# sdiehl/sonic

Hardware: AMD Instinct MI355X
Metric: prove() proofs/sec (higher is better)
Workload: dtype u32 limbs (Fq 12x32, Fr 8x32 Montgomery); 1 GPU; prove(): rndCircuit n=2^18, Q=2, SRS d=2^21 (d=8n >= 7n, Protocol.hs:54); n=262144, Q=2, d=2097152, process_group=none (plain single-process run), legs=headline only (the other legs: --full)

## Files before the change

sonic_amd/csrc/msm.hip:

```cpp
#include <string.h>
#include <stdexcept>
#include "internal.hpp"
#include "g1_quad.hpp"
#include "endo.hpp"

namespace sonic {

#ifndef SONIC_PART_LOW_BITS
#define SONIC_PART_LOW_BITS 8
#endif
constexpr int PART_LOW_BITS = SONIC_PART_LOW_BITS;
#ifndef SONIC_PART_TILE
#define SONIC_PART_TILE 1024
#endif
constexpr int PART_TILE = SONIC_PART_TILE;
constexpr uint32_t PASS1_GRID = 1024;
constexpr uint32_t PART_SORT_GRID = 2048;
#ifndef SONIC_PART_SORT_THREADS
#define SONIC_PART_SORT_THREADS 1024
#endif
constexpr int PART_SORT_THREADS = SONIC_PART_SORT_THREADS;
#ifndef SONIC_PART_SCATTER_THREADS
#define SONIC_PART_SCATTER_THREADS 512
#endif
// ... 36 lines not shown
  p.nseg = p.NB / K;
}

MsmPlan msm_plan(long n, bool fold) {
  MsmPlan p;
  p.fold = fold;
  int lg = 0;
  while ((1L << (lg + 1)) <= n) lg++;
  int c = lg - 4;
  if (c < 4) c = 4;
  if (c > 16) c = 16;
  if (g_window_override >= 4 && g_window_override <= 16) c = g_window_override;
  p.c = c;
  p.W = ((fold ? 255 : 256) + c - 1) / c;
  p.Wb = p.W;
  p.table_stride = 0;
  plan_finish(p, n);
  return p;
}

MsmPlan msm_plan_tables(long n, int c, int W, long table_stride, bool endo) {
  MsmPlan p;
  p.fold = true;
  p.endo = endo;
  p.bits = endo ? ENDO_BITS : 255;
  p.c = c;
  p.W = W;
  p.Wb = 1;
  p.table_stride = table_stride;
  plan_finish(p, n);
  return p;
}

void MsmWorkspace::reserve(long n, const MsmPlan& pl, int k) {
  const size_t sets = (size_t)k * pl.Wb;
  size_t M = sets * pl.NB;
  size_t NW = (size_t)n * pl.W;
  const size_t part_hn = (size_t)ceil_div((long)pl.Wb * pl.NB, 1L << PART_LOW_BITS) * (size_t)(ceil_div(n, PART_TILE) + k);
  count.ensure((2 * part_hn + 4) * 4);
  off.ensure((M + 1) * 4);
  digits.ensure(NW * 8);
  entries.ensure(NW * 4);
  buckets.ensure(M * sizeof(G1XYZZ));
  segres.ensure((sets * pl.nseg + sets * (pl.nseg / 256 + 1) + 2) * sizeof(G1XYZZ));
  scan_tmp.ensure((part_hn / 2048 + 4) * 4);
  order.ensure((M + 1) * 4);
  size_t max_heavy = NW / pl.heavy_threshold + 1;
  heavy_meta.ensure(sizeof(HeavyMeta) + max_heavy * sizeof(HeavyRec));
  heavy_partial.ensure((max_heavy + HEAVY_GRID + 1) * sizeof(G1XYZZ));
}

__device__ __forceinline__ bool fr_gt_half(const Fr& s) {
  constexpr uint32_t half[8] = FR_HALF;
#pragma unroll
  for (int i = 7; i >= 0; i--) {
    if (s.l[i] > half[i]) return true;
    if (s.l[i] < half[i]) return false;
  }
  return false;
}

__device__ __forceinline__ uint32_t block_exclusive_scan_256(uint32_t v, uint32_t* sh, uint32_t* total);
__device__ __forceinline__ uint32_t size_class(uint32_t sz) { return 255u - (sz < 255u ? sz : 255u); }


struct MsmBatchDev {
  int k;
  int bits;
  int slot_off[MSM_MAX_JOBS];
  int slot_form;
  uint32_t tile0[MSM_MAX_JOBS + 1];
  const char* points[MSM_MAX_JOBS];
  uint32_t pt_stride;
  long tstride[MSM_MAX_JOBS];
  const Fr* scalars[MSM_MAX_JOBS];
  long n[MSM_MAX_JOBS];
  MsmSlot* slot[MSM_MAX_JOBS];
// ... 523 lines not shown
      acc = k == (uint32_t)q ? c : g1q_add(acc, c, cr);
    }
    reinterpret_cast<Fq*>(&sh[q])[cr] = acc;
    __syncthreads();
    for (int sp = 8; sp >= 1; sp >>= 1) {
      if (q < sp && (uint32_t)(q + sp) < r.npart) {
        Fq* pa = reinterpret_cast<Fq*>(&sh[q]) + cr;
        *pa = g1q_add(*pa, reinterpret_cast<const Fq*>(&sh[q + sp])[cr], cr);
      }
      __syncthreads();
    }
    if (threadIdx.x < 4) reinterpret_cast<Fq*>(&buckets[r.bucket])[threadIdx.x] = reinterpret_cast<const Fq*>(&sh[0])[threadIdx.x];
    __syncthreads();
  }
}

#ifndef SONIC_SEGMENTS_LDS_TOT
#define SONIC_SEGMENTS_LDS_TOT 1
#endif
struct LdsPoint {
  uint32_t* base;
  __device__ __forceinline__ void store(const G1XYZZ& p) const {
    const uint32_t* w = reinterpret_cast<const uint32_t*>(&p);
#pragma unroll
    for (int k = 0; k < 48; k++) base[k * 256] = w[k];
  }
  __device__ __forceinline__ G1XYZZ load() const {
    G1XYZZ p;
    uint32_t* w = reinterpret_cast<uint32_t*>(&p);
#pragma unroll
    for (int k = 0; k < 48; k++) w[k] = base[k * 256];
    return p;
  }
};
__global__ __launch_bounds__(256, SONIC_SEGMENTS_LDS_TOT ? 2 : 1) void k_bucket_segments(const G1XYZZ* __restrict__ buckets, int W, int NB, int K, int nseg, int sg_base,
                                                        G1XYZZ* __restrict__ segres) {
#if SONIC_SEGMENTS_LDS_TOT
  __shared__ uint32_t tot_sh[48 * 256];
  const LdsPoint tl{tot_sh + threadIdx.x};
#endif
  int t = blockIdx.x * blockDim.x + threadIdx.x;
  if (t >= W * nseg) return;
  const int w = t / nseg, sl = t % nseg;
  const G1XYZZ* B = buckets + (size_t)w * NB + (size_t)sl * K;
  const int sg = sg_base + sl;
  const int k0 = sg * K;
  G1XYZZ run = G1XYZZ::inf();
#if SONIC_SEGMENTS_LDS_TOT
  tl.store(G1XYZZ::inf());
  for (int j = K - 1; j >= 0; j--) {
    run = g1_add(run, B[j]);
    tl.store(g1_add(tl.load(), run));
  }
#else
  G1XYZZ tot = G1XYZZ::inf();
  for (int j = K - 1; j >= 0; j--) {
    run = g1_add(run, B[j]);
    tot = g1_add(tot, run);
  }
#endif
  G1XYZZ acc = G1XYZZ::inf();
  bool have_multiple = false;
  if (nseg % 64 == 0 && sg_base % 64 == 0) {
    const uint32_t hi = __builtin_amdgcn_readfirstlane((uint32_t)sg >> 6), lo = (uint32_t)sg & 63u;
    for (int i = 31 - __clz((int)(hi | 1u)); i >= 0; i--) {
      acc = g1_dbl(acc);
      if ((hi >> i) & 1u) acc = g1_add(acc, run);
    }
    for (int i = 5; i >= 0; i--) {
      acc = g1_dbl(acc);
      if ((lo >> i) & 1u) acc = g1_add(acc, run);
    }
    for (int s = K; s > 1; s >>= 1) acc = g1_dbl(acc);
    have_multiple = true;
  } else if (k0) {
    acc = g1_mul_small(run, (uint32_t)k0);
    have_multiple = true;
  }
#if SONIC_SEGMENTS_LDS_TOT
  G1XYZZ tot = tl.load();
#endif
  if (have_multiple) tot = g1_add(tot, acc);
  segres[t] = tot;
}

__global__ __launch_bounds__(256, 2) void k_window_sum(const G1XYZZ* __restrict__ segres, int W, int c, int nseg, const MsmBatchDev batch) {
  __shared__ G1XYZZ sh[256];
  const int w = blockIdx.x % W;
  MsmSlot* slot = batch.slot[blockIdx.x / W];
  segres += (size_t)(blockIdx.x - w) * nseg;
  G1XYZZ acc = G1XYZZ::inf();
  for (int s = threadIdx.x; s < nseg; s += 256) acc = g1_add(acc, segres[(size_t)w * nseg + s]);
  sh[threadIdx.x] = acc;
  __syncthreads();
  for (int s = 128; s >= 1; s >>= 1) {
    if ((int)threadIdx.x < s) sh[threadIdx.x] = g1_add(sh[threadIdx.x], sh[threadIdx.x + s]);
    __syncthreads();
  }
  if (threadIdx.x == 0) {
    G1XYZZ r = sh[0];
    r.x = fp_canonical(r.x); r.y = fp_canonical(r.y); r.zz = fp_canonical(r.zz); r.zzz = fp_canonical(r.zzz);
    slot->win[w] = r;
    if (w == 0) { slot->W = W; slot->c = c; slot->pad0 = 0; slot->pad1 = 0; }
  }
}

__global__ __launch_bounds__(256, 2) void k_group_sum(const G1XYZZ* __restrict__ in, long n_in, int group, G1XYZZ* __restrict__ out) {
  __shared__ G1XYZZ sh[256];
  const long base = (long)blockIdx.x * group;
  G1XYZZ acc = G1XYZZ::inf();
  for (long s = threadIdx.x; s < group && base + s < n_in; s += 256) acc = g1_add(acc, in[base + s]);
  sh[threadIdx.x] = acc;
  __syncthreads();
  for (int s = 128; s >= 1; s >>= 1) {
    if ((int)threadIdx.x < s) sh[threadIdx.x] = g1_add(sh[threadIdx.x], sh[threadIdx.x + s]);
    __syncthreads();
  }
  if (threadIdx.x == 0) out[blockIdx.x] = sh[0];
}

constexpr int TREE_BLOCK_LOG = 10;
constexpr int TREE_MID_LOG = 14;
#ifndef SONIC_TREE_LATENCY_MAX
#define SONIC_TREE_LATENCY_MAX (1L << 17)
#endif
constexpr long TREE_LATENCY_MAX_BUCKETS = SONIC_TREE_LATENCY_MAX;
constexpr int TREE_LATENCY_BLOCK_LOG = 7, TREE_LATENCY_MID_LOG = 12;

__device__ __forceinline__ void tree_item(G1XYZZ* __restrict__ Z, size_t s0, int m, uint32_t it) {
  const uint32_t pair = it / (uint32_t)m, comp = it % (uint32_t)m;
  const size_t s = s0 + ((size_t)pair << m);
  const size_t pos = comp == 0 ? 0 : (size_t)1 << (comp - 1);
  const size_t h = (size_t)1 << (m - 1);
  Z[s + pos] = g1_add(Z[s + pos], Z[s + h + pos]);
// ... 23 lines not shown
  const bool leaf_in_registers = quads < 32;
  if (!leaf_in_registers) {
    tree_level(Z, s0, 1, 1u << (LB - 1), quads);
    __syncthreads();
    tree_level(Z, s0, 2, 2u << (LB - 2), quads);
  } else if (threadIdx.x < nthreads) {
    G1XYZZ* b = Z + s0 + 4 * (size_t)threadIdx.x;
    const G1XYZZ odd = g1_add(b[1], b[3]);
    const G1XYZZ p23 = g1_add(b[2], b[3]);
    b[3] = odd;
    const G1XYZZ tot = g1_add(g1_add(b[0], b[1]), p23);
    b[2] = p23;
    b[0] = tot;
    b[1] = b[3];
  }
  for (int m = 3; m <= LB; m++) {
    __syncthreads();
    tree_level(Z, s0, m, (uint32_t)m << (LB - m), quads);
  }
}

template <int THREADS>
__global__ __launch_bounds__(THREADS, THREADS == 256 ? 2 : 1) void k_bucket_tree_levels(G1XYZZ* __restrict__ Z, int span_log, int m_lo, int m_hi, int final_L,
                                                               uint32_t tot_mul, int quads, const MsmBatchDev batch) {
  const size_t s0 = (size_t)blockIdx.x << span_log;
  for (int m = m_lo; m <= m_hi; m++) {
    if (m > m_lo) __syncthreads();
    tree_level(Z, s0, m, (uint32_t)m << (span_log - m), quads);
  }
  if (final_L > 0) {
    __syncthreads();
    MsmSlot* slot = batch.slot[blockIdx.x];
    const int off = batch.slot_off[blockIdx.x];
    if ((int)threadIdx.x <= final_L) {
      G1XYZZ r = Z[s0 + ((int)threadIdx.x == final_L ? 0 : (size_t)1 << threadIdx.x)];
      r.x = fp_canonical(r.x); r.y = fp_canonical(r.y); r.zz = fp_canonical(r.zz); r.zzz = fp_canonical(r.zzz);
      slot->win[off + threadIdx.x] = r;
    }
    if (threadIdx.x == 0 && off == 0) { slot->W = final_L; slot->c = 1; slot->pad0 = (int)tot_mul; slot->pad1 = batch.slot_form; }
  }
}


static void bucket_tree_enqueue(hipStream_t st, G1XYZZ* Z, int sets, int L, uint32_t tot_mul, const MsmBatchDev& batch) {
  if (((long)sets << L) <= TREE_LATENCY_MAX_BUCKETS) {
    constexpr int all_quads = 1 << 20;
    const int LB = L < TREE_LATENCY_BLOCK_LOG ? L : TREE_LATENCY_BLOCK_LOG;
    LAUNCH(k_bucket_tree_block, (uint32_t)sets << (L - LB), 256, 0, st, Z, LB, all_quads);
    int done = LB;
    if (L > TREE_LATENCY_MID_LOG) {
      LAUNCH(k_bucket_tree_levels<512>, (uint32_t)sets << (L - TREE_LATENCY_MID_LOG), 512, 0, st, Z, TREE_LATENCY_MID_LOG, done + 1, TREE_LATENCY_MID_LOG, 0, 0u, all_quads, batch);
      done = TREE_LATENCY_MID_LOG;
    }
    LAUNCH(k_bucket_tree_levels<512>, (uint32_t)sets, 512, 0, st, Z, L, done + 1, L, L, tot_mul, all_quads, batch);
    return;
  }
  const int LB = L < TREE_BLOCK_LOG ? L : TREE_BLOCK_LOG;
  constexpr int quads = 2;
  LAUNCH(k_bucket_tree_block, (uint32_t)sets << (L - LB), 256, 0, st, Z, LB, quads);
  int done = LB;
  if (L > done) {
    const int mid = L < TREE_MID_LOG ? L : TREE_MID_LOG;
    if (mid < L) {
      LAUNCH(k_bucket_tree_levels<256>, (uint32_t)sets << (L - mid), 256, 0, st, Z, mid, done + 1, mid, 0, 0u, quads, batch);
      done = mid;
    }
  }
  LAUNCH(k_bucket_tree_levels<256>, (uint32_t)sets, 256, 0, st, Z, L, done + 1, L, L, tot_mul, quads, batch);
}

G1XYZZ msm_finish_host(const MsmSlot& s) {
  const int W = s.W, c = s.c;
  G1XYZZ acc = G1XYZZ::inf();
  if (s.pad1 == 1 || s.pad1 == 2) {
    auto bitsum = [&](int off) {
      G1XYZZ a = G1XYZZ::inf();
      for (int w = W - 1; w >= 0; w--) {
        G1XYZZ win;
        memcpy(&win, &s.win[off + w], sizeof win);
        a = g1_add(g1_dbl(a), win);
      }
      G1XYZZ tot;
      memcpy(&tot, &s.win[off + W], sizeof tot);
      const uint32_t mul = (uint32_t)s.pad0;
      return g1_add(a, mul == 1 ? tot : g1_mul_small(tot, mul));
    };
    if (s.pad1 == 1) return bitsum(0);
    return g1_add(bitsum(0), g1_endo(bitsum(MSM_ENDO_SLOT_OFFSET)));
  }
  for (int w = W - 1; w >= 0; w--) {
    G1XYZZ win;
    memcpy(&win, &s.win[w], sizeof win);
    if (w == W - 1) { acc = win; continue; }
    for (int j = 0; j < c; j++) acc = g1_dbl(acc);
    acc = g1_add(acc, win);
  }
  return acc;
}
bool msm_can_batch(const MsmPlan& pl) { return pl.Wb == 1 && pl.NB >= (1 << PART_LOW_BITS); }

__global__ __launch_bounds__(256) void k_endo_split(const Fr* __restrict__ sc, long n, int mont, Fr* __restrict__ s1, Fr* __restrict__ s2) {
  const long i = (long)blockIdx.x * blockDim.x + threadIdx.x;
  if (i >= n) return;
  Fr s = sc[i];
  if (mont) s = fp_from_mont(s);
  Fr a, b;
  endo_split(s, a, b);
  s1[i] = a; s2[i] = b;
}

void msm_enqueue_batch(hipStream_t st, MsmWorkspace& ws, const MsmPlan& pl, const MsmJob* jobs, int k, bool scalars_mont, G1XYZZ* ext_buckets) {
  if (k < 1 || k > MSM_MAX_JOBS) throw std::runtime_error("msm_enqueue_batch: 1..MSM_MAX_JOBS jobs");
  if (ext_buckets && (k != 1 || pl.Wb != 1)) throw std::runtime_error("msm_enqueue_batch: bucket hand-off needs one job over a shared bucket set");
  if (k > 1 && !msm_can_batch(pl)) throw std::runtime_error("msm_enqueue_batch: plan cannot be batched");
  MsmJob split_jobs[MSM_MAX_JOBS];
  bool fold = pl.fold;
  if (pl.endo) {
    if (ext_buckets) { set_error("the bucket hand-off of a bucket-sharded MSM needs the full window tables (this SRS holds endomorphism tables)"); throw HipFail{SONIC_ERR_INVALID_ARG}; }
    if (2 * k > MSM_MAX_JOBS) {
      const int h = MSM_MAX_JOBS / 2;
      for (int j0 = 0; j0 < k; j0 += h) msm_enqueue_batch(st, ws, pl, jobs + j0, k - j0 < h ? k - j0 : h, scalars_mont, nullptr);
      return;
    }
    long n_all = 0;
    for (int j = 0; j < k; j++) n_all += jobs[j].n;
    ws.endo_scalars.ensure(sizeof(Fr) * 2 * (size_t)(n_all > 0 ? n_all : 1));
    Fr* halves = ws.endo_scalars.as<Fr>();
    for (int j = 0; j < k; j++) {
      Fr* s1 = halves; Fr* s2 = halves + jobs[j].n;
      halves += 2 * jobs[j].n;
      if (jobs[j].n > 0) LAUNCH(k_endo_split, ceil_div(jobs[j].n, 256), 256, 0, st, jobs[j].scalars, jobs[j].n, (int)scalars_mont, s1, s2);
// ... 76 lines not shown
      const long mean = nmax * pl.W / (P > 0 ? P : 1);
      stage_cap = 2048;
      while (stage_cap < 32768 && (long)stage_cap < mean + mean / 2) stage_cap *= 2;
    }
    LAUNCH(k_part_sort, nparts < PART_SORT_GRID ? nparts : PART_SORT_GRID, PART_SORT_THREADS, (size_t)stage_cap * 4, st, batch, (const uint2*)ws.digits.as<uint2>(),
           (const uint32_t*)hbase, (const uint32_t*)total, hn, P, jobstride, off, ws.entries.as<uint32_t>(), hm->class_hist, stage_cap);
  }
  LAUNCH(k_border_place, ceil_div((long)M, 2048), 256, 0, st, (const uint32_t*)off, (uint32_t)M, (const uint32_t*)hm->class_hist, hm->class_cursor,
         ws.order.as<uint32_t>());
  const int accum_block = (pl.accum_block == 64 || pl.accum_block == 128) ? pl.accum_block : 256;
  static const int split_env = getenv("SONIC_ACCUM_LANES") ? atoi(getenv("SONIC_ACCUM_LANES")) : 0;
  const int lanes_per_bucket = split_env == 1 ? 1 : (M <= 65536 ? 4 : (M <= 131072 ? 2 : 1));
  if (lanes_per_bucket == 4)
    LAUNCH(k_bucket_accum_split<4>, ceil_div(4 * (long)M, 256), 256, 0, st, batch, jobstride, (const uint32_t*)ws.entries.as<uint32_t>(),
           (const uint32_t*)off, (const uint32_t*)ws.order.as<uint32_t>(), (uint32_t)M, pl.heavy_threshold, buckets, hm, hrecs);
  else if (lanes_per_bucket == 2)
    LAUNCH(k_bucket_accum_split<2>, ceil_div(2 * (long)M, 256), 256, 0, st, batch, jobstride, (const uint32_t*)ws.entries.as<uint32_t>(),
           (const uint32_t*)off, (const uint32_t*)ws.order.as<uint32_t>(), (uint32_t)M, pl.heavy_threshold, buckets, hm, hrecs);
  else
  LAUNCH(k_bucket_accum, ceil_div((long)M, accum_block), accum_block, 0, st, batch, jobstride, (const uint32_t*)ws.entries.as<uint32_t>(),
         (const uint32_t*)off, (const uint32_t*)ws.order.as<uint32_t>(), (uint32_t)M, pl.heavy_threshold, buckets, hm, hrecs);
  LAUNCH(k_heavy_accum, HEAVY_GRID, HEAVY_THREADS, 0, st, batch, jobstride, (const uint32_t*)ws.entries.as<uint32_t>(), (const uint32_t*)off,
         (const HeavyMeta*)hm, hrecs, ws.heavy_partial.as<G1XYZZ>());
  LAUNCH(k_heavy_finish, HEAVY_GRID / 2, 64, 0, st, (const HeavyMeta*)hm, (const HeavyRec*)hrecs,
         (const G1XYZZ*)ws.heavy_partial.as<G1XYZZ>(), buckets);
  if (ext_buckets) return;
  const int sets = k * pl.Wb;
  if ((pl.tree && pl.Wb == 1 && pl.NB >= 4) || pl.endo) {
    int L = 0;
    while ((1 << L) < pl.NB) L++;
    bucket_tree_enqueue(st, ws.buckets.as<G1XYZZ>(), sets, L, 1u, batch);
    return;
  }
  LAUNCH(k_bucket_segments, ceil_div((long)sets * pl.nseg, 256), 256, 0, st, (const G1XYZZ*)ws.buckets.as<G1XYZZ>(), sets,
         pl.NB, pl.K, pl.nseg, 0, ws.segres.as<G1XYZZ>());
  if (pl.nseg > 4096) {
    const int group = 256, ngroups = pl.nseg / group;
    G1XYZZ* part = ws.segres.as<G1XYZZ>() + (size_t)sets * pl.nseg;
    LAUNCH(k_group_sum, sets * ngroups, 256, 0, st, (const G1XYZZ*)ws.segres.as<G1XYZZ>(), (long)sets * pl.nseg, group, part);
    LAUNCH(k_window_sum, sets, 256, 0, st, (const G1XYZZ*)part, pl.Wb, pl.c, ngroups, batch);
  } else {
    LAUNCH(k_window_sum, sets, 256, 0, st, (const G1XYZZ*)ws.segres.as<G1XYZZ>(), pl.Wb, pl.c, pl.nseg, batch);
  }
}

__global__ __launch_bounds__(256, 1) void k_sum_slices(const G1XYZZ* __restrict__ slices, int k, long len, G1XYZZ* __restrict__ out) {
  const long i = (long)blockIdx.x * blockDim.x + threadIdx.x;
  if (i >= len) return;
  G1XYZZ acc = slices[i];
  for (int s = 1; s < k; s++) acc = g1_add(acc, slices[(size_t)s * len + i]);
  out[i] = acc;
}

void msm_reduce_slices_enqueue(hipStream_t st, MsmWorkspace& ws, const G1XYZZ* d_slices, int k, long len, long base, int c, MsmSlot* d_slot) {
  (void)c;
  if (k < 1 || len < 4 || len % MSM_SLICE_QUANTUM || base % MSM_SLICE_QUANTUM || base + len >= (1L << 31))
    throw std::runtime_error("msm_reduce_slices_enqueue: slice length and base must be multiples of MSM_SLICE_QUANTUM");
  int L = 2;
  while (((long)1 << L) < len) L++;
  const long P = (long)1 << L;
  ws.buckets.ensure((size_t)P * sizeof(G1XYZZ));
  if (P > len) HIP_OK(hipMemsetAsync(ws.buckets.as<G1XYZZ>() + len, 0, (size_t)(P - len) * sizeof(G1XYZZ), st));
  LAUNCH(k_sum_slices, ceil_div(len, 256), 256, 0, st, d_slices, k, len, ws.buckets.as<G1XYZZ>());
  MsmBatchDev b1;
  memset(&b1, 0, sizeof b1);
  b1.k = 1;
  b1.bits = 255;
  b1.slot_form = 1;
  b1.slot[0] = d_slot;
  bucket_tree_enqueue(st, ws.buckets.as<G1XYZZ>(), 1, L, (uint32_t)(base + 1), b1);
}

void msm_enqueue(hipStream_t st, MsmWorkspace& ws, const MsmPlan& pl, PointArray d_points, const Fr* d_scalars,
                 long n, bool scalars_mont, MsmSlot* d_slot) {
  MsmJob job{d_points, d_scalars, n, d_slot};
// ... 5 lines not shown
```

sonic_amd/csrc/msm.hpp:

```cpp
#pragma once
#include "common.hpp"
#include "g1.hpp"
#include "g1_host.hpp"

namespace sonic {

HD int msm_even_width(int W, int w, int bits = 255) { return bits / W + (w < bits % W ? 1 : 0); }
HD int msm_even_shift(int W, int w, int bits = 255) { const int base = bits / W, extra = bits % W; return w * base + (w < extra ? w : extra); }

struct MsmPlan {
  int c;
  int W;
  int Wb;
  long table_stride;
  int NB;
  int K;
  int nseg;
  uint32_t heavy_threshold;
  int accum_block = 256;
  bool tree = true;
  bool endo = false;
  int bits = 255;
  bool fold;
};
MsmPlan msm_plan(long n, bool fold = true);
MsmPlan msm_plan_tables(long n, int c, int W, long table_stride, bool endo = false);
void msm_plan_set_segment(MsmPlan& p, int K);

constexpr int MSM_MAX_WINDOWS = 64;
constexpr long MSM_TABLE_MAX_TERMS = 1L << 26;
constexpr int MSM_TABLE_MAX_WINDOWS = 32;
constexpr long MSM_MAX_TERMS = 1L << 31;

struct MsmSlot {
  int W, c, pad0, pad1;
  G1XYZZ win[MSM_MAX_WINDOWS];
};

struct MsmWorkspace {
  DevBuf count, off, digits, entries, buckets, segres, scan_tmp, order, heavy_meta, heavy_partial, endo_scalars;
  void reserve(long n, const MsmPlan& pl, int k = 1);
};

void msm_enqueue(hipStream_t st, MsmWorkspace& ws, const MsmPlan& pl, PointArray d_points,
                 const Fr* d_scalars, long n, bool scalars_mont, MsmSlot* d_slot);

constexpr int MSM_MAX_JOBS = 16;
constexpr int MSM_ENDO_SLOT_OFFSET = 32;
struct MsmJob { PointArray points; const Fr* scalars; long n; MsmSlot* slot; long table_stride = 0; };
bool msm_can_batch(const MsmPlan& pl);
void msm_enqueue_batch(hipStream_t st, MsmWorkspace& ws, const MsmPlan& pl, const MsmJob* jobs, int k, bool scalars_mont,
                       G1XYZZ* ext_buckets = nullptr);
constexpr long MSM_SLICE_QUANTUM = 16384;
void msm_reduce_slices_enqueue(hipStream_t st, MsmWorkspace& ws, const G1XYZZ* d_slices, int k, long len, long base, int c, MsmSlot* d_slot);

G1XYZZ msm_finish_host(const MsmSlot& s);
int msm_window_override();
void msm_set_window_override(int c);

}
```

sonic_amd/csrc/msm_api.hip:

```cpp
#include <string.h>
#include <condition_variable>
#include <memory>
#include <string>
#include <vector>
#include "srs_handle.hpp"

using namespace sonic;

extern "C" {

int sonic_msm_set_window(int c) { msm_set_window_override(c); return SONIC_OK; }

int sonic_msm_plan(const sonic_srs_t* srs, int64_t n, int* window_bits, int* windows, int* bucket_sets) {
  if (!srs || n < 0) return SONIC_ERR_INVALID_ARG;
  if (n >= MSM_MAX_TERMS) { set_error("MSM of %ld terms: at most 2^31 - 1 (entry encoding)", (long)n); return SONIC_ERR_INVALID_ARG; }
  MsmPlan pl = srs_msm_plan(srs, n);
  if (window_bits) *window_bits = pl.c;
  if (windows) *windows = pl.W;
  if (bucket_sets) *bucket_sets = pl.Wb;
  return SONIC_OK;
}

int sonic_msm_g1(const uint8_t* points, const uint8_t* scalars, int64_t n, uint8_t out_g1[96]) {
  API_BEGIN
// ... 333 lines not shown
      }
  if (exchange) return sonic_g1_sum_dev_partials(blobs.data(), world, out_g1);
  G1XYZZ acc = G1XYZZ::inf();
  for (int r = 0; r < world; r++) acc = g1_add(acc, partial[(size_t)r]);
  g1_canonical_bytes_host(acc, out_g1);
  return SONIC_OK;
}

int sonic_msm_g1_srs_multi_dev(const sonic_srs_t* const* srs, int world, int basis, const int64_t* e0, const void* const* d_scalars, const int64_t* n, int mode,
                               uint8_t out_g1[96]) {
  if (!e0 || !d_scalars || !n) return SONIC_ERR_INVALID_ARG;
  try { return msm_multi(srs, world, basis, e0, d_scalars, nullptr, n, mode, out_g1); }
  catch (const std::exception& e) { set_error("%s", e.what()); return SONIC_ERR_HIP; }
}
int sonic_msm_g1_srs_multi(const sonic_srs_t* const* srs, int world, int basis, int64_t e0, const uint8_t* scalars, int64_t n, int mode, uint8_t out_g1[96]) {
  if (world < 1 || world > 64 || n < 0 || (n > 0 && !scalars)) return SONIC_ERR_INVALID_ARG;
  std::vector<int64_t> e((size_t)world), cnt((size_t)world);
  std::vector<const uint8_t*> hs((size_t)world);
  for (int r = 0; r < world; r++) {
    const int64_t lo = n * r / world, hi = n * (r + 1) / world;
    e[(size_t)r] = e0 + lo; cnt[(size_t)r] = hi - lo; hs[(size_t)r] = scalars + 32 * (size_t)lo;
  }
  try { return msm_multi(srs, world, basis, e.data(), nullptr, hs.data(), cnt.data(), mode, out_g1); }
  catch (const std::exception& e2) { set_error("%s", e2.what()); return SONIC_ERR_HIP; }
}

static_assert(sizeof(MsmSlot) == SONIC_G1_DEV_PARTIAL_BYTES, "SONIC_G1_DEV_PARTIAL_BYTES is the size of a device-side MSM result");
int sonic_g1_sum_dev_partials(const uint8_t* blobs, int k, uint8_t out_g1[96]) {
  if (!blobs || k < 1 || !out_g1) return SONIC_ERR_INVALID_ARG;
  G1XYZZ acc = G1XYZZ::inf();
  std::unique_ptr<MsmSlot> s(new MsmSlot());
  for (int i = 0; i < k; i++) {
    memcpy(s.get(), blobs + sizeof(MsmSlot) * (size_t)i, sizeof(MsmSlot));
    if (s->W < 0 || s->W > MSM_MAX_WINDOWS || (s->pad1 == 1 && s->W >= MSM_MAX_WINDOWS) || (s->pad1 == 2 && s->W >= MSM_MAX_WINDOWS - MSM_ENDO_SLOT_OFFSET) || s->pad1 < 0 || s->pad1 > 2 || s->c < 0 || s->c > 32) { set_error("sonic_g1_sum_dev_partials: blob %d is not a device-side MSM result", i); return SONIC_ERR_INVALID_ARG; }
    acc = g1_add(acc, msm_finish_host(*s));
  }
  g1_canonical_bytes_host(acc, out_g1);
  return SONIC_OK;
}

int sonic_g1_sum_partials(const uint8_t* partials, int k, uint8_t out_g1[96]) {
  if (!partials || k < 1 || !out_g1) return SONIC_ERR_INVALID_ARG;
  G1XYZZ acc = G1XYZZ::inf();
  for (int i = 0; i < k; i++) { G1XYZZ p; memcpy(&p, partials + sizeof(G1XYZZ) * i, sizeof p); acc = g1_add(acc, p); }
  g1_canonical_bytes_host(acc, out_g1);
  return SONIC_OK;
}

}
```

sonic_amd/csrc/prove.hip:

```cpp
#include "prover.hpp"
#include "witness_tree.hpp"

namespace sonic {

static int prove_segment(const MsmPlan& pl, int k, bool last) {
  const bool big = pl.NB >= (1 << 18);
  if (last) return big ? 16 : 4;
  return k > 1 ? (big ? 64 : 16) : (big ? 8 : 4);
}

MsmJob commit_job(hipStream_t st, const sonic_srs* srs, const Fr* poly, long lo, long len, long maxm, MsmSlot* slot, int* d_flags) {
  const long d = srs->d, shift = d - maxm;
  long i0 = -d - shift - lo, i1 = d - shift - lo + 1;
  if (i0 < 0) i0 = 0;
  if (i1 > len) i1 = len;
  if (i1 < i0) i1 = i0;
  flag_nonzero_enqueue(st, poly, i0, d_flags, FLAG_SRS_INDEX);
  flag_nonzero_enqueue(st, poly + i1, len - i1, d_flags, FLAG_SRS_INDEX);
  const long ih = -shift - lo;
  if (ih >= i0 && ih < i1) flag_nonzero_enqueue(st, poly + ih, 1, d_flags, FLAG_SRS_INDEX);
  return MsmJob{srs->basis(1) + (lo + i0 + shift + d), poly + i0, i1 - i0, slot};
}

void run_jobs(hipStream_t st, const sonic_srs* srs, MsmWorkspace& ws, const MsmJob* jobs, int k, bool last, bool exposed) {
  if (k <= 0) return;
  long nmax = 0;
  for (int j = 0; j < k; j++) nmax = std::max(nmax, jobs[j].n);
  MsmPlan pl = srs_msm_plan(srs, nmax);
  const bool tree = last || exposed || pl.NB <= (1 << 17);
  if (k > 1 && msm_can_batch(pl)) {
    msm_plan_set_segment(pl, prove_segment(pl, k, last));
    pl.tree = tree;
    msm_enqueue_batch(st, ws, pl, jobs, k, true);
    return;
  }
  for (int j = 0; j < k; j++) {
    MsmPlan p1 = srs_msm_plan(srs, jobs[j].n);
    msm_plan_set_segment(p1, prove_segment(p1, 1, false));
    p1.tree = tree;
    msm_enqueue_batch(st, ws, p1, &jobs[j], 1, true);
  }
}

static void eval_prefix_enqueue(hipStream_t st, Scratch& sc, const Fr* poly, long lo, long len, const Fr* zpair, Fr* d_fz) {
  sc.reserve(len);
  sc.scan.ensure(sizeof(Fr) * (len / 1024 + 2));
  poly_scale_powers_enqueue(st, poly, sc.D.as<Fr>(), len, lo, zpair, zpair + 1);
  poly_prefix_sum_enqueue(st, sc.D.as<Fr>(), len, sc.scan);
  HIP_OK(hipMemcpyAsync(d_fz, sc.D.as<Fr>() + (len - 1), sizeof(Fr), hipMemcpyDeviceToDevice, st));
}

static MsmJob quotient_job(hipStream_t st, const sonic_srs* srs, const Fr* q, long lo, long len, MsmSlot* slot, int* d_flags) {
  const long d = srs->d, qn = len - 1;
  long i0 = -d - lo, i1 = d - lo + 1;
  if (i0 < 0) i0 = 0;
  if (i1 > qn) i1 = qn;
  if (i1 < i0) i1 = i0;
  flag_nonzero_enqueue(st, q, i0, d_flags, FLAG_SRS_INDEX);
  flag_nonzero_enqueue(st, q + i1, qn - i1, d_flags, FLAG_SRS_INDEX);
  return MsmJob{srs->basis(0) + (lo + i0 + d), q + i0, i1 - i0, slot};
}

MsmJob open_job(hipStream_t st, const sonic_srs* srs, Scratch& sc, const Fr* poly, long lo, long len,
                       const Fr* zpair, Fr* d_fz, MsmSlot* slot, int* d_flags) {
  sc.reserve(len);
  eval_prefix_enqueue(st, sc, poly, lo, len, zpair, d_fz ? d_fz : sc.fz_discard.as<Fr>());
  poly_quotient_enqueue(st, sc.D.as<Fr>(), sc.q.as<Fr>(), len, lo, zpair, zpair + 1);
  return quotient_job(st, srs, sc.q.as<Fr>(), lo, len, slot, d_flags);
}

MsmJob open_job_at_zero(hipStream_t st, const sonic_srs* srs, const Fr* poly, long len, Fr* d_fz, MsmSlot* slot, int* d_flags) {
// ... 731 lines not shown
      memcpy(&lo, b + 8 * i, 4); memcpy(&hi, b + 8 * i + 4, 4);
      if (hi <= lo) continue;
      pieces.push_back({lo, hi});
      G1XYZZ part;
      memcpy(&part, b + 8 * K + 192 * (size_t)i, 192);
      sums[(size_t)i] = g1_add(sums[(size_t)i], part);
    }
    std::sort(pieces.begin(), pieces.end());
    uint32_t at = 0;
    for (auto& pc : pieces) { if (pc.first != at) break; at = pc.second; }
    if (at != SHARE_ONE) { set_error("sonic_proof_from_shares: the pieces of MSM %d do not cover its terms exactly once", i); return SONIC_ERR_INVALID_ARG; }
  }
  std::vector<uint8_t> pts(96 * (size_t)K), frs(32 * (size_t)F);
  g1_canonical_bytes_host_batch(sums.data(), K, pts.data());
  for (int i = 0; i < F; i++) {
    bool got = false;
    for (int r = 0; r < world && !got; r++) {
      const uint8_t* b = by_rank[(size_t)r] + sizeof(ShareHeader) + 8 * (size_t)K + 192 * (size_t)K;
      int32_t v; memcpy(&v, b + 32 * (size_t)F + 4 * (size_t)i, 4);
      if (v) { memcpy(&frs[32 * (size_t)i], b + 32 * (size_t)i, 32); got = true; }
    }
    if (!got) { set_error("sonic_proof_from_shares: no share reports evaluation %d", i); return SONIC_ERR_INVALID_ARG; }
  }
  proof_layout(Q, pts.data(), frs.data(), transcript, out_proof);
  } catch (const std::exception& e) { set_error("%s", e.what()); return SONIC_ERR_HIP; }
  return SONIC_OK;
}

static bool slots_folded(const MsmSlot* hs, long K) {
  for (long i = 0; i < K; i++) if (hs[i].W > 1 && hs[i].pad1 == 0) return false;
  return true;
}
static void finish_slots_host(const MsmSlot* hs, long K, G1XYZZ* out, int max_threads) {
  const int nt = slots_folded(hs, K) ? 1 : (int)std::min<long>(K, max_threads);
  ThreadGroup th;
  for (int w = 1; w < nt; w++) th.emplace_back([=] { for (long i = w; i < K; i += nt) out[i] = msm_finish_host(hs[i]); });
  for (long i = 0; i < K; i += nt) out[i] = msm_finish_host(hs[i]);
}

static int prove_finish(sonic_prover_t* p, uint8_t* out_proof) {
  API_BEGIN_ON(p->device)
  const long Q = p->Q;
  const ProofLayout L{Q};
  const int K = (int)L.K();
  const uint8_t* transcript = p->h_tr;
  const bool timing = await_proof(p, false);
  const MsmSlot* hs = p->h_slots;
  const uint8_t* hfr_p = p->h_fr;
  const int hflags = *p->h_flags;
  if (p->h_flags[1]) { p->have_assignment = false; return flags_to_status(p->h_flags[1], "prove (circuit / assignment handed over with the call)"); }
  if (hflags) return flags_to_status(hflags, "prove");
  std::vector<uint8_t> pts(96 * (size_t)K);
  {
    auto t0 = std::chrono::steady_clock::now();
    std::vector<G1XYZZ> sums((size_t)K);
    const bool has_extra = p->prepared || p->runs_on;
    std::vector<G1XYZZ> side((size_t)(Q + 1), G1XYZZ::inf());
    const MsmSlot* hx = hs + L.S_extra(0);
    ThreadGroup th;
    if (p->sym_on) th.emplace_back([&] { side[(size_t)Q] = msm_finish_host(hs[L.C_extra()]); });
    if (has_extra && !slots_folded(hx, Q)) th.emplace_back([&] { finish_slots_host(hx, Q, side.data(), 8); });
    else if (has_extra) finish_slots_host(hx, Q, side.data(), 1);
    finish_slots_host(hs, K, sums.data(), 16);
    th.join();
    fold_side_slots(L, has_extra, p->sym_on, sums.data(), side.data(), g1_sum);
    g1_canonical_bytes_host_batch(sums.data(), K, pts.data());
    if (timing) fprintf(stderr, "[sonic] host tails of %d MSMs: %.3f ms\n", K, std::chrono::duration<double, std::milli>(std::chrono::steady_clock::now() - t0).count());
// ... 547 lines not shown
```

Measured before the change: 28.46 proofs/s.

## Reduce MSM segment prefix multiples via two-level bucket tree instead of per-segment scalar muls

For batched prove MSMs with large bucket counts, the segment kernel now emits each segment's running sum separately and skips the per-segment double-and-add by the segment index. Those runs are combined by the existing bucket tree into bit-weighted windows, and a new slot form (pad1=3) tells the host finisher to apply the doublings for segment size K and add the total. The segment size drops to 32 in this mode, and the LDS total accumulation now does a mixed add in place instead of a load/add/store round trip. This trades many per-thread scalar multiplications for an extra tree launch, a larger segres buffer, and more host finishing work, which is spread across up to 4 threads.

```diff
diff --git a/sonic_amd/csrc/msm.hip b/sonic_amd/csrc/msm.hip
--- a/sonic_amd/csrc/msm.hip
+++ b/sonic_amd/csrc/msm.hip
@@ -92,6 +92,8 @@
   return p;
 }
 
+static size_t segres_runs_offset(size_t sets, int nseg) { return sets * nseg + sets * (nseg / 256 + 1) + 2; }
+
 void MsmWorkspace::reserve(long n, const MsmPlan& pl, int k) {
   const size_t sets = (size_t)k * pl.Wb;
   size_t M = sets * pl.NB;
@@ -102,7 +104,7 @@
   digits.ensure(NW * 8);
   entries.ensure(NW * 4);
   buckets.ensure(M * sizeof(G1XYZZ));
-  segres.ensure((sets * pl.nseg + sets * (pl.nseg / 256 + 1) + 2) * sizeof(G1XYZZ));
+  segres.ensure((segres_runs_offset(sets, pl.nseg) + (pl.two_level && pl.Wb == 1 ? sets * pl.nseg : 0)) * sizeof(G1XYZZ));
   scan_tmp.ensure((part_hn / 2048 + 4) * 4);
   order.ensure((M + 1) * 4);
   size_t max_heavy = NW / pl.heavy_threshold + 1;
@@ -692,25 +694,57 @@
     for (int k = 0; k < 48; k++) w[k] = base[k * 256];
     return p;
   }
+  __device__ __forceinline__ Fq coord(int i) const {
+    Fq f;
+#pragma unroll
+    for (int k = 0; k < 12; k++) f.l[k] = base[(12 * i + k) * 256];
+    return f;
+  }
+  __device__ __forceinline__ void set_coord(int i, const Fq& f) const {
+#pragma unroll
+    for (int k = 0; k < 12; k++) base[(12 * i + k) * 256] = f.l[k];
+  }
+  __device__ __forceinline__ void add(const G1XYZZ& q) const {
+    if (q.is_inf()) return;
+    const Fq pzz = coord(2);
+    if (pzz.is_zero_strict()) { store(q); return; }
+    const Fq U1 = fp_mul(coord(0), q.zz);
+    const Fq U2 = fp_mul(q.x, pzz);
+    const Fq S1 = fp_mul(coord(1), q.zzz);
+    const Fq S2 = fp_mul(q.y, coord(3));
+    const Fq Pp = fp_sub(U2, U1);
+    const Fq R = fp_sub(S2, S1);
+    if (Pp.is_zero()) {
+      store(R.is_zero() ? g1_dbl(load()) : G1XYZZ::inf());
+      return;
+    }
+    const Fq PP = fp_sqr(Pp);
+    const Fq PPP = fp_mul(Pp, PP);
+    const Fq Qv = fp_mul(U1, PP);
+    const Fq x = fp_sub(fp_sub(fp_sqr(R), PPP), fp_dbl(Qv));
+    set_coord(0, x);
+    set_coord(1, fp_sub(fp_mul(R, fp_sub(Qv, x)), fp_mul(S1, PPP)));
+    set_coord(2, fp_mul(fp_mul(coord(2), q.zz), PP));
+    set_coord(3, fp_mul(fp_mul(coord(3), q.zzz), PPP));
+  }
 };
-__global__ __launch_bounds__(256, SONIC_SEGMENTS_LDS_TOT ? 2 : 1) void k_bucket_segments(const G1XYZZ* __restrict__ buckets, int W, int NB, int K, int nseg, int sg_base,
-                                                        G1XYZZ* __restrict__ segres) {
+template <bool RUNS>
+__global__ __launch_bounds__(256, SONIC_SEGMENTS_LDS_TOT ? 2 : 1) void k_bucket_segments(const G1XYZZ* __restrict__ buckets, int W, int NB, int K, int nseg,
+                                                        G1XYZZ* __restrict__ segres, G1XYZZ* __restrict__ runs) {
 #if SONIC_SEGMENTS_LDS_TOT
   __shared__ uint32_t tot_sh[48 * 256];
   const LdsPoint tl{tot_sh + threadIdx.x};
 #endif
   int t = blockIdx.x * blockDim.x + threadIdx.x;
   if (t >= W * nseg) return;
-  const int w = t / nseg, sl = t % nseg;
-  const G1XYZZ* B = buckets + (size_t)w * NB + (size_t)sl * K;
-  const int sg = sg_base + sl;
-  const int k0 = sg * K;
+  const int w = t / nseg, sg = t % nseg;
+  const G1XYZZ* B = buckets + (size_t)w * NB + (size_t)sg * K;
   G1XYZZ run = G1XYZZ::inf();
 #if SONIC_SEGMENTS_LDS_TOT
   tl.store(G1XYZZ::inf());
   for (int j = K - 1; j >= 0; j--) {
     run = g1_add(run, B[j]);
-    tl.store(g1_add(tl.load(), run));
+    tl.add(run);
   }
 #else
   G1XYZZ tot = G1XYZZ::inf();
@@ -719,9 +753,19 @@
     tot = g1_add(tot, run);
   }
 #endif
+  if (RUNS) {
+    runs[t] = run;
+#if SONIC_SEGMENTS_LDS_TOT
+    segres[t] = tl.load();
+#else
+    segres[t] = tot;
+#endif
+    return;
+  }
+  const int k0 = sg * K;
   G1XYZZ acc = G1XYZZ::inf();
   bool have_multiple = false;
-  if (nseg % 64 == 0 && sg_base % 64 == 0) {
+  if (nseg % 64 == 0) {
     const uint32_t hi = __builtin_amdgcn_readfirstlane((uint32_t)sg >> 6), lo = (uint32_t)sg & 63u;
     for (int i = 31 - __clz((int)(hi | 1u)); i >= 0; i--) {
       acc = g1_dbl(acc);
@@ -744,7 +788,7 @@
   segres[t] = tot;
 }
 
-__global__ __launch_bounds__(256, 2) void k_window_sum(const G1XYZZ* __restrict__ segres, int W, int c, int nseg, const MsmBatchDev batch) {
+__global__ __launch_bounds__(256, 2) void k_window_sum(const G1XYZZ* __restrict__ segres, int W, int c, int nseg, int runs_L, int K, const MsmBatchDev batch) {
   __shared__ G1XYZZ sh[256];
   const int w = blockIdx.x % W;
   MsmSlot* slot = batch.slot[blockIdx.x / W];
@@ -760,6 +804,7 @@
   if (threadIdx.x == 0) {
     G1XYZZ r = sh[0];
     r.x = fp_canonical(r.x); r.y = fp_canonical(r.y); r.zz = fp_canonical(r.zz); r.zzz = fp_canonical(r.zzz);
+    if (runs_L > 0) { slot->win[runs_L] = r; slot->W = runs_L; slot->c = 1; slot->pad0 = K; slot->pad1 = 3; return; }
     slot->win[w] = r;
     if (w == 0) { slot->W = W; slot->c = c; slot->pad0 = 0; slot->pad1 = 0; }
   }
@@ -849,12 +894,12 @@
     __syncthreads();
     MsmSlot* slot = batch.slot[blockIdx.x];
     const int off = batch.slot_off[blockIdx.x];
-    if ((int)threadIdx.x <= final_L) {
+    if ((int)threadIdx.x < final_L + (tot_mul != 0u ? 1 : 0)) {
       G1XYZZ r = Z[s0 + ((int)threadIdx.x == final_L ? 0 : (size_t)1 << threadIdx.x)];
       r.x = fp_canonical(r.x); r.y = fp_canonical(r.y); r.zz = fp_canonical(r.zz); r.zzz = fp_canonical(r.zzz);
       slot->win[off + threadIdx.x] = r;
     }
-    if (threadIdx.x == 0 && off == 0) { slot->W = final_L; slot->c = 1; slot->pad0 = (int)tot_mul; slot->pad1 = batch.slot_form; }
+    if (threadIdx.x == 0 && off == 0 && tot_mul != 0u) { slot->W = final_L; slot->c = 1; slot->pad0 = (int)tot_mul; slot->pad1 = batch.slot_form; }
   }
 }
 
@@ -886,34 +931,6 @@
   LAUNCH(k_bucket_tree_levels<256>, (uint32_t)sets, 256, 0, st, Z, L, done + 1, L, L, tot_mul, quads, batch);
 }
 
-G1XYZZ msm_finish_host(const MsmSlot& s) {
-  const int W = s.W, c = s.c;
-  G1XYZZ acc = G1XYZZ::inf();
-  if (s.pad1 == 1 || s.pad1 == 2) {
-    auto bitsum = [&](int off) {
-      G1XYZZ a = G1XYZZ::inf();
-      for (int w = W - 1; w >= 0; w--) {
-        G1XYZZ win;
-        memcpy(&win, &s.win[off + w], sizeof win);
-        a = g1_add(g1_dbl(a), win);
-      }
-      G1XYZZ tot;
-      memcpy(&tot, &s.win[off + W], sizeof tot);
-      const uint32_t mul = (uint32_t)s.pad0;
-      return g1_add(a, mul == 1 ? tot : g1_mul_small(tot, mul));
-    };
-    if (s.pad1 == 1) return bitsum(0);
-    return g1_add(bitsum(0), g1_endo(bitsum(MSM_ENDO_SLOT_OFFSET)));
-  }
-  for (int w = W - 1; w >= 0; w--) {
-    G1XYZZ win;
-    memcpy(&win, &s.win[w], sizeof win);
-    if (w == W - 1) { acc = win; continue; }
-    for (int j = 0; j < c; j++) acc = g1_dbl(acc);
-    acc = g1_add(acc, win);
-  }
-  return acc;
-}
 bool msm_can_batch(const MsmPlan& pl) { return pl.Wb == 1 && pl.NB >= (1 << PART_LOW_BITS); }
 
 __global__ __launch_bounds__(256) void k_endo_split(const Fr* __restrict__ sc, long n, int mont, Fr* __restrict__ s1, Fr* __restrict__ s2) {
@@ -1056,15 +1073,24 @@
     bucket_tree_enqueue(st, ws.buckets.as<G1XYZZ>(), sets, L, 1u, batch);
     return;
   }
-  LAUNCH(k_bucket_segments, ceil_div((long)sets * pl.nseg, 256), 256, 0, st, (const G1XYZZ*)ws.buckets.as<G1XYZZ>(), sets,
-         pl.NB, pl.K, pl.nseg, 0, ws.segres.as<G1XYZZ>());
+  int runs_L = 0;
+  if (pl.two_level && pl.Wb == 1 && pl.nseg >= 4) while ((1 << runs_L) < pl.nseg) runs_L++;
+  if (runs_L > 0) {
+    G1XYZZ* runs = ws.segres.as<G1XYZZ>() + segres_runs_offset(sets, pl.nseg);
+    LAUNCH(k_bucket_segments<true>, ceil_div((long)sets * pl.nseg, 256), 256, 0, st, (const G1XYZZ*)ws.buckets.as<G1XYZZ>(), sets,
+           pl.NB, pl.K, pl.nseg, ws.segres.as<G1XYZZ>(), runs);
+    bucket_tree_enqueue(st, runs, sets, runs_L, 0u, batch);
+  } else {
+    LAUNCH(k_bucket_segments<false>, ceil_div((long)sets * pl.nseg, 256), 256, 0, st, (const G1XYZZ*)ws.buckets.as<G1XYZZ>(), sets,
+           pl.NB, pl.K, pl.nseg, ws.segres.as<G1XYZZ>(), (G1XYZZ*)nullptr);
+  }
   if (pl.nseg > 4096) {
     const int group = 256, ngroups = pl.nseg / group;
     G1XYZZ* part = ws.segres.as<G1XYZZ>() + (size_t)sets * pl.nseg;
     LAUNCH(k_group_sum, sets * ngroups, 256, 0, st, (const G1XYZZ*)ws.segres.as<G1XYZZ>(), (long)sets * pl.nseg, group, part);
-    LAUNCH(k_window_sum, sets, 256, 0, st, (const G1XYZZ*)part, pl.Wb, pl.c, ngroups, batch);
+    LAUNCH(k_window_sum, sets, 256, 0, st, (const G1XYZZ*)part, pl.Wb, pl.c, ngroups, runs_L, pl.K, batch);
   } else {
-    LAUNCH(k_window_sum, sets, 256, 0, st, (const G1XYZZ*)ws.segres.as<G1XYZZ>(), pl.Wb, pl.c, pl.nseg, batch);
+    LAUNCH(k_window_sum, sets, 256, 0, st, (const G1XYZZ*)ws.segres.as<G1XYZZ>(), pl.Wb, pl.c, pl.nseg, runs_L, pl.K, batch);
   }
 }
 
diff --git a/sonic_amd/csrc/msm.hpp b/sonic_amd/csrc/msm.hpp
--- a/sonic_amd/csrc/msm.hpp
+++ b/sonic_amd/csrc/msm.hpp
@@ -2,6 +2,7 @@
 #include "common.hpp"
 #include "g1.hpp"
 #include "g1_host.hpp"
+#include "msm_slot.hpp"
 
 namespace sonic {
 
@@ -19,6 +20,7 @@
   uint32_t heavy_threshold;
   int accum_block = 256;
   bool tree = true;
+  bool two_level = false;
   bool endo = false;
   int bits = 255;
   bool fold;
@@ -27,15 +29,9 @@
 MsmPlan msm_plan_tables(long n, int c, int W, long table_stride, bool endo = false);
 void msm_plan_set_segment(MsmPlan& p, int K);
 
-constexpr int MSM_MAX_WINDOWS = 64;
 constexpr long MSM_TABLE_MAX_TERMS = 1L << 26;
 constexpr int MSM_TABLE_MAX_WINDOWS = 32;
 constexpr long MSM_MAX_TERMS = 1L << 31;
-
-struct MsmSlot {
-  int W, c, pad0, pad1;
-  G1XYZZ win[MSM_MAX_WINDOWS];
-};
 
 struct MsmWorkspace {
   DevBuf count, off, digits, entries, buckets, segres, scan_tmp, order, heavy_meta, heavy_partial, endo_scalars;
@@ -46,7 +42,6 @@
                  const Fr* d_scalars, long n, bool scalars_mont, MsmSlot* d_slot);
 
 constexpr int MSM_MAX_JOBS = 16;
-constexpr int MSM_ENDO_SLOT_OFFSET = 32;
 struct MsmJob { PointArray points; const Fr* scalars; long n; MsmSlot* slot; long table_stride = 0; };
 bool msm_can_batch(const MsmPlan& pl);
 void msm_enqueue_batch(hipStream_t st, MsmWorkspace& ws, const MsmPlan& pl, const MsmJob* jobs, int k, bool scalars_mont,
@@ -54,7 +49,6 @@
 constexpr long MSM_SLICE_QUANTUM = 16384;
 void msm_reduce_slices_enqueue(hipStream_t st, MsmWorkspace& ws, const G1XYZZ* d_slices, int k, long len, long base, int c, MsmSlot* d_slot);
 
-G1XYZZ msm_finish_host(const MsmSlot& s);
 int msm_window_override();
 void msm_set_window_override(int c);
 
diff --git a/sonic_amd/csrc/msm_api.hip b/sonic_amd/csrc/msm_api.hip
--- a/sonic_amd/csrc/msm_api.hip
+++ b/sonic_amd/csrc/msm_api.hip
@@ -389,7 +389,7 @@
   std::unique_ptr<MsmSlot> s(new MsmSlot());
   for (int i = 0; i < k; i++) {
     memcpy(s.get(), blobs + sizeof(MsmSlot) * (size_t)i, sizeof(MsmSlot));
-    if (s->W < 0 || s->W > MSM_MAX_WINDOWS || (s->pad1 == 1 && s->W >= MSM_MAX_WINDOWS) || (s->pad1 == 2 && s->W >= MSM_MAX_WINDOWS - MSM_ENDO_SLOT_OFFSET) || s->pad1 < 0 || s->pad1 > 2 || s->c < 0 || s->c > 32) { set_error("sonic_g1_sum_dev_partials: blob %d is not a device-side MSM result", i); return SONIC_ERR_INVALID_ARG; }
+    if (s->W < 0 || s->W > MSM_MAX_WINDOWS || (s->pad1 == 1 && s->W >= MSM_MAX_WINDOWS) || (s->pad1 == 2 && s->W >= MSM_MAX_WINDOWS - MSM_ENDO_SLOT_OFFSET) || (s->pad1 == 3 && (s->W >= MSM_MAX_WINDOWS || s->pad0 < 1 || (s->pad0 & (s->pad0 - 1)))) || s->pad1 < 0 || s->pad1 > 3 || s->c < 0 || s->c > 32) { set_error("sonic_g1_sum_dev_partials: blob %d is not a device-side MSM result", i); return SONIC_ERR_INVALID_ARG; }
     acc = g1_add(acc, msm_finish_host(*s));
   }
   g1_canonical_bytes_host(acc, out_g1);
diff --git a/sonic_amd/csrc/msm_slot.hpp b/sonic_amd/csrc/msm_slot.hpp
--- /dev/null
+++ b/sonic_amd/csrc/msm_slot.hpp
@@ -0,0 +1,57 @@
+#pragma once
+#include <string.h>
+#include "g1.hpp"
+#include "endo.hpp"
+
+namespace sonic {
+
+constexpr int MSM_MAX_WINDOWS = 64;
+constexpr int MSM_ENDO_SLOT_OFFSET = 32;
+
+struct MsmSlot {
+  int W, c, pad0, pad1;
+  G1XYZZ win[MSM_MAX_WINDOWS];
+};
+
+inline G1XYZZ msm_finish_host(const MsmSlot& s) {
+  const int W = s.W, c = s.c;
+  G1XYZZ acc = G1XYZZ::inf();
+  if (s.pad1 >= 1 && s.pad1 <= 3) {
+    auto bitsum = [&](int off) {
+      G1XYZZ a = G1XYZZ::inf();
+      for (int w = W - 1; w >= 0; w--) {
+        G1XYZZ win;
+        memcpy(&win, &s.win[off + w], sizeof win);
+        a = g1_add(g1_dbl(a), win);
+      }
+      G1XYZZ tot;
+      memcpy(&tot, &s.win[off + W], sizeof tot);
+      const uint32_t mul = (uint32_t)s.pad0;
+      return g1_add(a, mul == 1 ? tot : g1_mul_small(tot, mul));
+    };
+    if (s.pad1 == 1) return bitsum(0);
+    if (s.pad1 == 3) {
+      G1XYZZ a = G1XYZZ::inf();
+      for (int w = W - 1; w >= 0; w--) {
+        G1XYZZ win;
+        memcpy(&win, &s.win[w], sizeof win);
+        a = g1_add(g1_dbl(a), win);
+      }
+      for (uint32_t k = (uint32_t)s.pad0; k > 1; k >>= 1) a = g1_dbl(a);
+      G1XYZZ tot;
+      memcpy(&tot, &s.win[W], sizeof tot);
+      return g1_add(a, tot);
+    }
+    return g1_add(bitsum(0), g1_endo(bitsum(MSM_ENDO_SLOT_OFFSET)));
+  }
+  for (int w = W - 1; w >= 0; w--) {
+    G1XYZZ win;
+    memcpy(&win, &s.win[w], sizeof win);
+    if (w == W - 1) { acc = win; continue; }
+    for (int j = 0; j < c; j++) acc = g1_dbl(acc);
+    acc = g1_add(acc, win);
+  }
+  return acc;
+}
+
+}
diff --git a/sonic_amd/csrc/prove.hip b/sonic_amd/csrc/prove.hip
--- a/sonic_amd/csrc/prove.hip
+++ b/sonic_amd/csrc/prove.hip
@@ -3,10 +3,21 @@
 
 namespace sonic {
 
-static int prove_segment(const MsmPlan& pl, int k, bool last) {
+constexpr long PROVE_TWO_LEVEL_MAX_TERMS = 1L << 21;
+static bool prove_two_level(const MsmPlan& pl, int k, bool last, long nmax) {
+  if (last || k <= 1 || pl.NB < (1 << 18)) return false;
+  const char* e = getenv("SONIC_PROVE_TWO_LEVEL");
+  if (e && (e[0] == '0' || e[0] == '1') && !e[1]) return e[0] == '1';
+  return nmax <= PROVE_TWO_LEVEL_MAX_TERMS;
+}
+static int prove_segment(const MsmPlan& pl, int k, bool last, bool two_level) {
   const bool big = pl.NB >= (1 << 18);
   if (last) return big ? 16 : 4;
-  return k > 1 ? (big ? 64 : 16) : (big ? 8 : 4);
+  if (k <= 1) return big ? 8 : 4;
+  if (!big) return 16;
+  const char* e = getenv("SONIC_PROVE_SEGMENT");
+  const int v = e ? atoi(e) : 0;
+  return v >= 8 && v <= 1024 ? v : (two_level ? 32 : 64);
 }
 
 MsmJob commit_job(hipStream_t st, const sonic_srs* srs, const Fr* poly, long lo, long len, long maxm, MsmSlot* slot, int* d_flags) {
@@ -29,14 +40,15 @@
   MsmPlan pl = srs_msm_plan(srs, nmax);
   const bool tree = last || exposed || pl.NB <= (1 << 17);
   if (k > 1 && msm_can_batch(pl)) {
-    msm_plan_set_segment(pl, prove_segment(pl, k, last));
+    pl.two_level = prove_two_level(pl, k, last, nmax);
+    msm_plan_set_segment(pl, prove_segment(pl, k, last, pl.two_level));
     pl.tree = tree;
     msm_enqueue_batch(st, ws, pl, jobs, k, true);
     return;
   }
   for (int j = 0; j < k; j++) {
     MsmPlan p1 = srs_msm_plan(srs, jobs[j].n);
-    msm_plan_set_segment(p1, prove_segment(p1, 1, false));
+    msm_plan_set_segment(p1, prove_segment(p1, 1, false, false));
     p1.tree = tree;
     msm_enqueue_batch(st, ws, p1, &jobs[j], 1, true);
   }
@@ -834,7 +846,9 @@
   return true;
 }
 static void finish_slots_host(const MsmSlot* hs, long K, G1XYZZ* out, int max_threads) {
-  const int nt = slots_folded(hs, K) ? 1 : (int)std::min<long>(K, max_threads);
+  long two_level = 0;
+  for (long i = 0; i < K; i++) two_level += hs[i].pad1 == 3;
+  const int nt = !slots_folded(hs, K) ? (int)std::min<long>(K, max_threads) : (two_level >= 8 ? std::min(4, max_threads) : 1);
   ThreadGroup th;
   for (int w = 1; w < nt; w++) th.emplace_back([=] { for (long i = w; i < K; i += nt) out[i] = msm_finish_host(hs[i]); });
   for (long i = 0; i < K; i += nt) out[i] = msm_finish_host(hs[i]);
```

Result: faster. 29.86 proofs/s, median of 6 (+4.9%).
